# lighttransport/nanort

Measured on AMD Instinct MI355X. Metric: Mrays/s (primary + 1-bounce) at 1920x1080, 1M-tri mesh; BVH build ms, higher is better.
Workload: dtype f32; 1 GPU; C3: Plane(1000,500) = 1,000,000 triangles fp32; 1920x1080 objrender-camera primaries + 1 cosine bounce per hit (2073600 + 2055142 rays per GPU per step); parallelism=replicated BVH, interleaved image rows per GPU

## Files before the change

include/nanort_hip.h:

```cpp
#ifndef NANORT_HIP_H_
#define NANORT_HIP_H_

#include <stddef.h>
#include <stdint.h>

#ifdef __cplusplus
extern "C" {
#endif

#define NRT_API __attribute__((visibility("default")))

typedef int nrt_status;
enum {
  NRT_OK = 0,
  NRT_ERR_INVALID = 1,
  NRT_ERR_EMPTY = 2,
  NRT_ERR_DEVICE = 3,
  NRT_ERR_PRECISION = 4
};

typedef struct nrt_ctx nrt_ctx;


typedef struct {
// ... 92 lines not shown
#endif


NRT_API nrt_status nrtCreate(int device, nrt_ctx **out);
NRT_API void nrtDestroy(nrt_ctx *ctx);
NRT_API const char *nrtLastError(const nrt_ctx *ctx);
NRT_API const char *nrtVersion(void);

NRT_API nrt_status nrtHostAlloc(size_t bytes, void **out);
NRT_API void nrtHostFree(void *p);

NRT_API nrt_status nrtSetMesh_f32(nrt_ctx *ctx, const float *vertices, size_t vertex_stride_bytes,
                                  const uint32_t *faces, uint32_t num_faces);
NRT_API nrt_status nrtSetMesh_f64(nrt_ctx *ctx, const double *vertices, size_t vertex_stride_bytes,
                                  const uint32_t *faces, uint32_t num_faces);

NRT_API nrt_status nrtOccludedBatch_f32(nrt_ctx *ctx, const nrt_ray_f32 *rays, uint64_t num_rays,
                                        const nrt_trace_options *options, uint8_t *mask_out);
NRT_API nrt_status nrtOccludedBatch_f64(nrt_ctx *ctx, const nrt_ray_f64 *rays, uint64_t num_rays,
                                        const nrt_trace_options *options, uint8_t *mask_out);
NRT_API nrt_status nrtOccludedBatchDevice_f32(nrt_ctx *ctx, const nrt_ray_f32 *d_rays, uint64_t num_rays,
                                              const nrt_trace_options *options, uint8_t *d_mask_out, void *hip_stream);
NRT_API nrt_status nrtOccludedBatchDevice_f64(nrt_ctx *ctx, const nrt_ray_f64 *d_rays, uint64_t num_rays,
                                              const nrt_trace_options *options, uint8_t *d_mask_out, void *hip_stream);

#define NRT_MAX_MULTIHIT 64u
NRT_API nrt_status nrtMultiHitTraverseBatch_f32(nrt_ctx *ctx, const nrt_ray_f32 *rays, uint64_t num_rays, uint32_t max_hits,
                                                const nrt_trace_options *options, nrt_hit_f32 *hits_out, uint32_t *counts_out);
NRT_API nrt_status nrtMultiHitTraverseBatch_f64(nrt_ctx *ctx, const nrt_ray_f64 *rays, uint64_t num_rays, uint32_t max_hits,
                                                const nrt_trace_options *options, nrt_hit_f64 *hits_out, uint32_t *counts_out);
// ... 155 lines not shown
```

nanort_amd/accel.py:

```python
import ctypes

import numpy as np

from . import capi
from .wire import (
    BUILD_OPTIONS_F32,
    BUILD_OPTIONS_F64,
    BUILD_STATS,
    TRACE_OPTIONS,
    hit_dtype,
    node_dtype,
    ray_dtype,
    suffix,
)


def _p(a):
    return None if a is None else a.ctypes.data_as(ctypes.c_void_p)


class TriangleMesh:

    def __init__(self, vertices, faces, vertex_stride_bytes=None):
        self.vertices = np.ascontiguousarray(vertices)
# ... 79 lines not shown
        if isinstance(mesh, SphereGeometry):
            if self.real != np.float32:
                raise TypeError("sphere primitives are fp32 (as the reference example)")
            self._check(self._L.nrtSetSpheres_f32(self._h, _p(mesh.centers), _p(mesh.radii), mesh.num_spheres))
            self._mesh = mesh
            return
        if mesh.vertices.dtype != self.real:
            raise TypeError("mesh precision %s != accel precision %s" % (mesh.vertices.dtype, self.real))
        self._check(
            getattr(self._L, "nrtSetMesh_" + self._s)(
                self._h, _p(mesh.vertices), mesh.vertex_stride_bytes, _p(mesh.faces), mesh.num_faces
            )
        )
        self._mesh = mesh

    def Build(self, num_primitives, mesh, options=None):
        if num_primitives != mesh.num_faces:
            if isinstance(mesh, CylinderGeometry):
                mesh = CylinderGeometry(mesh.endpoints[:num_primitives], mesh.radii[:num_primitives], mesh.test_cap)
            elif isinstance(mesh, SphereGeometry):
                mesh = SphereGeometry(mesh.centers[:num_primitives], mesh.radii[:num_primitives])
            else:
                mesh = TriangleMesh(mesh.vertices, mesh.faces[:num_primitives], mesh.vertex_stride_bytes)
        self.SetMesh(mesh)
        if options is not None:
            want = BUILD_OPTIONS_F32 if self.real == np.float32 else BUILD_OPTIONS_F64
            options = np.asarray(options, dtype=want).reshape(1)
        nn = ctypes.c_uint64(0)
        st = getattr(self._L, "nrtBuild_" + self._s)(self._h, _p(options), _p(self._stats.reshape(1)), ctypes.byref(nn))
        if st == capi.NRT_ERR_EMPTY:
            return False
        self._check(st)
        return True

    def GetStatistics(self):
        return self._stats.copy()

    def LastBuildMs(self):
        return float(self._L.nrtLastBuildMs(self._h))
# ... 335 lines not shown
```

nanort_amd/capi.py:

```python
import ctypes
import os

_HERE = os.path.dirname(os.path.abspath(__file__))
LIB_PATH = os.path.join(_HERE, "lib", "libnanort_hip_prof.so" if os.environ.get("NRT_USE_PROF_LIB") == "1" else "libnanort_hip.so")

NRT_OK, NRT_ERR_INVALID, NRT_ERR_EMPTY, NRT_ERR_DEVICE, NRT_ERR_PRECISION = 0, 1, 2, 3, 4

SYMBOLS = [
    "nrtCreate", "nrtDestroy", "nrtLastError", "nrtVersion",
    "nrtSetMesh_f32", "nrtSetMesh_f64", "nrtSetSpheres_f32",
    "nrtSetCylinders_f32", "nrtTraverseBatchCylinders_f32", "nrtTraverseBatchCylindersDevice_f32",
    "nrtBuild_f32", "nrtBuild_f64",
    "nrtGetTree_f32", "nrtGetTree_f64", "nrtTreeSize", "nrtGetTreeBounds_f32", "nrtGetTreeBounds_f64",
    "nrtSetTree_f32", "nrtSetTree_f64",
    "nrtTraverseBatch_f32", "nrtTraverseBatch_f64",
    "nrtTraverseBatchDevice_f32", "nrtTraverseBatchDevice_f64", "nrtTraverseBatchesDevice_f32", "nrtTraverseBatchesDevice_f64", "nrtTraverseBatches_f32", "nrtTraverseBatches_f64",
    "nrtTraverseBatchMulti_f32", "nrtTraverseBatchMulti_f64", "nrtDeviceCount",
    "nrtTraverseCountDevice_f32", "nrtTraverseCountDevice_f64",
    "nrtOccludedBatch_f32", "nrtOccludedBatch_f64", "nrtOccludedBatchDevice_f32", "nrtOccludedBatchDevice_f64",
    "nrtMultiHitTraverseBatch_f32", "nrtMultiHitTraverseBatch_f64", "nrtMultiHitTraverseBatchDevice_f32", "nrtMultiHitTraverseBatchDevice_f64",
    "nrtRefit_f32", "nrtRefit_f64", "nrtRefitDevice_f32", "nrtRefitDevice_f64",
    "nrtLastTraverseMs", "nrtSetLaunchTiming", "nrtSetTunable", "nrtGetTunable", "nrtLastBuildMs", "nrtLastKernelName", "nrtHostAlloc", "nrtHostFree",
    "nrtGroupUniqueId", "nrtGroupCreate", "nrtGroupCreateRanked", "nrtGroupDestroy", "nrtGroupLastError", "nrtGroupSetTunable", "nrtGroupInfo",
    "nrtGroupTileRays", "nrtGroupTraverseGather_f32", "nrtGroupTraverseGather_f64", "nrtGroupTraverseGatherTiles_f32", "nrtGroupTraverseGatherTiles_f64", "nrtGroupSynchronize", "nrtGroupLastTraffic",
    "nrtSceneCreate", "nrtSceneDestroy", "nrtSceneLastError", "nrtSceneAddNode_f32", "nrtSceneCommit", "nrtSceneNodeState_f32",
# ... 35 lines not shown
    L = ctypes.CDLL(LIB_PATH, mode=ctypes.RTLD_GLOBAL)
    vp, u32, u64, sz, i32 = ctypes.c_void_p, ctypes.c_uint32, ctypes.c_uint64, ctypes.c_size_t, ctypes.c_int
    L.nrtCreate.argtypes = [i32, ctypes.POINTER(vp)]
    L.nrtCreate.restype = i32
    L.nrtDestroy.argtypes = [vp]
    L.nrtDestroy.restype = None
    L.nrtLastError.argtypes = [vp]
    L.nrtLastError.restype = ctypes.c_char_p
    L.nrtVersion.argtypes = []
    L.nrtVersion.restype = ctypes.c_char_p
    L.nrtTreeSize.argtypes = [vp, ctypes.POINTER(u64), ctypes.POINTER(u64)]
    L.nrtTreeSize.restype = i32
    for s in ("f32", "f64"):
        f = getattr(L, "nrtSetMesh_" + s)
        f.argtypes = [vp, vp, sz, vp, u32]
        f.restype = i32
        f = getattr(L, "nrtBuild_" + s)
        f.argtypes = [vp, vp, vp, ctypes.POINTER(u64)]
        f.restype = i32
        f = getattr(L, "nrtGetTree_" + s)
        f.argtypes = [vp, vp, vp]
        f.restype = i32
        f = getattr(L, "nrtSetTree_" + s)
        f.argtypes = [vp, vp, u64, vp, u64]
        f.restype = i32
        f = getattr(L, "nrtTraverseBatch_" + s)
        f.argtypes = [vp, vp, u64, vp, vp, vp]
        f.restype = i32
        f = getattr(L, "nrtTraverseBatchDevice_" + s)
        f.argtypes = [vp, vp, u64, vp, vp, vp, vp]
# ... 85 lines not shown
```

nanort_amd/csrc/api.hip:

```cpp
#include <hip/hip_runtime.h>
#include <stdarg.h>
#include <stdio.h>
#include <stdlib.h>
#include <string.h>
#include <ctype.h>
#include <math.h>
#include <cmath>

#include <algorithm>
#include <atomic>
#include <chrono>
#include <mutex>
#include <thread>
#include <string>
#include <vector>

#include "common.h"
#ifdef NRT_PROF
#include "../../include/nanort_hip_prof.h"
#endif

namespace nrt {
template <typename T>
hipError_t launch_traverse(const TraverseArgs<T> &, unsigned grid, bool count, int lds_stack, hipStream_t);
template <typename T>
int traverse_blocks_per_cu(int lds_stack);
// ... 29 lines not shown
size_t refit_plan_bytes(uint32_t tree_depth, uint64_t num_nodes);
template <typename T>
hipError_t launch_refit_plan(const typename Wire<T>::Node *nodes, uint64_t num_nodes, uint32_t num_branch_records, uint32_t tree_depth,
                             uint32_t root_is_branch, uint32_t *plan, hipStream_t s);
template <typename T>
hipError_t launch_refit(const void *src, size_t stride, bool aligned, uint32_t nv, T *verts, const uint32_t *faces, const uint32_t *indices,
                        typename Wire<T>::Node *nodes, uint64_t num_nodes, uint32_t num_branch_records, uint32_t tree_depth,
                        const uint32_t *plan, hipStream_t s);
hipError_t launch_cylinder_segments(const float *verts, const float *radii, const uint32_t *seg_off, uint32_t n, float *seg_verts,
                                    float *seg_radii, uint32_t *seg_prim, hipStream_t s);
}

using namespace nrt;

static thread_local std::string g_create_error;

struct nrt_ctx {
  int device = 0;
  hipStream_t stream = nullptr;
  std::string err;
  int prec = 0;
  int num_cus = 256;

  int prim_kind = kPrimTriangles;
  uint32_t cyl_test_cap = 1;
  DevBuf b_seg_verts, b_seg_radii, b_seg_prim, b_seg_off;
  uint32_t num_segs = 0;
  int cyl_split = 32;
  int cyl_seg_radii = 8;
  DevBuf b_verts, b_radii, b_faces;
// ... 62 lines not shown
  unsigned static_pct = 16;
  unsigned static_bands = 8;
  unsigned static_slice_groups = 2;
  unsigned max_blocks_per_cu = 0;
  int wide = 1, wide_stack = 10;
  int wide4 = 1;
  int wide4_big_ok = 1;
  int order4 = 0;
  int leaf_compact = 1;
  int dyn_head = 1;
  int wide_scramble = 0;
  unsigned wide4_blocks_per_cu = 0;
  unsigned wide_blocks_per_cu = 0, sphere_blocks_per_cu = 0;
  unsigned multihit_blocks_per_cu = 0;

  hipEvent_t ev_b0 = nullptr, ev_b1 = nullptr;
  hipEvent_t ev_build_state = nullptr;
  void *build_state = nullptr;
  int last_timed_slot = -1;
  int launch_timing = 0;
  bool have_build_time = false;
  float segment_ms = 0.f;
  const char *last_kernel = "";
};

static nrt_status fail(nrt_ctx *c, nrt_status st, const char *fmt, ...) {
  char buf[512];
  va_list ap;
  va_start(ap, fmt);
  vsnprintf(buf, sizeof(buf), fmt, ap);
// ... 75 lines not shown
    if (e != hipSuccess) return e;
  }
  return hipStreamSynchronize(c->stream);
}

static void free_tree(nrt_ctx *c) {
  c->generation++;
  c->d_wide = nullptr;
  c->d_wide4 = nullptr;
  c->d_nodes = nullptr;
  c->d_indices = nullptr;
  c->d_tris = nullptr;
  c->num_nodes = c->num_indices = 0;
  c->tree_depth = 0;
  c->refit_planned = false;
}

static void free_mesh(nrt_ctx *c) {
  c->d_verts = nullptr;
  c->d_faces = nullptr;
  c->d_radii = nullptr;
  c->num_faces = c->num_verts = 0;
  c->num_segs = 0;
}

struct TunableDesc {
  const char *name;
  long long lo, hi;
  long long (*get)(const nrt_ctx *);
  void (*set)(nrt_ctx *, long long);
};
#define NRT_TUNABLE(name_, lo_, hi_, field_, type_)                                                          \
  {name_, lo_, hi_, [](const nrt_ctx *c) -> long long { return (long long)c->field_; },                      \
   [](nrt_ctx *c, long long v) { c->field_ = (type_)v; }}
static const TunableDesc kTunables[] = {
    NRT_TUNABLE("refill_min", 1, 64, refill_min, unsigned),
    NRT_TUNABLE("trav_min", 1, 64, trav_min, unsigned),
    NRT_TUNABLE("trav_min4", 1, 64, trav_min4, unsigned),
    NRT_TUNABLE("f64_row_fetch", 0, 1, f64_row_fetch, int),
    NRT_TUNABLE("leaf_min", 1, 64, leaf_min, unsigned),
    NRT_TUNABLE("chunk_tail_pct", 0, 100, chunk_tail_pct, unsigned),
    NRT_TUNABLE("parts", 1, kMaxParts, num_parts, unsigned),
    NRT_TUNABLE("static_pct", 0, 100, static_pct, unsigned),
    NRT_TUNABLE("static_bands", 1, 64, static_bands, unsigned),
    NRT_TUNABLE("static_slice_groups", 1, 64, static_slice_groups, unsigned),
    NRT_TUNABLE("blocks_per_cu", 0, 8, max_blocks_per_cu, unsigned),
    NRT_TUNABLE("debug", 0, 0x7FFFFFFF, debug_flags, unsigned),
    NRT_TUNABLE("morton", 0, 1, morton, int),
    NRT_TUNABLE("cyl_split", 1, 64, cyl_split, int),
    NRT_TUNABLE("cyl_seg_radii", 1, 1024, cyl_seg_radii, int),
#ifdef NRT_PROF
    NRT_TUNABLE("subtree_rows", 0, 1, subtree_rows, int),
#endif
    NRT_TUNABLE("wide", 0, 1, wide, int),
    NRT_TUNABLE("wide4_big", 0, 2, wide4_big_ok, int),
    NRT_TUNABLE("wide4", 0, 1, wide4, int),
    NRT_TUNABLE("leaf_compact", 0, 1, leaf_compact, int),
    NRT_TUNABLE("dyn_head", 0, 1, dyn_head, int),
    NRT_TUNABLE("order4", 0, 1, order4, int),
    NRT_TUNABLE("launch_timing", 0, 1, launch_timing, int),
    NRT_TUNABLE("host_pipeline", 0, 1, host_pipeline, int),
    NRT_TUNABLE("wide_scramble", 0, 1, wide_scramble, int),
// ... 45 lines not shown
  int ndev = 0;
  hipError_t e = hipGetDeviceCount(&ndev);
  if (e != hipSuccess || ndev <= 0)
    return fail(nullptr, NRT_ERR_DEVICE, "nrtCreate: no HIP device visible (%s)",
                e == hipSuccess ? "count == 0" : hipGetErrorString(e));
  if (device < 0 || device >= ndev)
    return fail(nullptr, NRT_ERR_INVALID, "nrtCreate: device %d out of range [0,%d)", device, ndev);
  nrt_ctx *c = new nrt_ctx();
  c->device = device;
  if ((e = hipSetDevice(device)) != hipSuccess ||
      (e = hipStreamCreateWithFlags(&c->stream, hipStreamNonBlocking)) != hipSuccess ||
      (e = hipEventCreate(&c->ev_b0)) != hipSuccess || (e = hipEventCreate(&c->ev_b1)) != hipSuccess ||
      (e = hipEventCreateWithFlags(&c->ev_build_state, hipEventDisableTiming)) != hipSuccess ||
      (e = hipEventCreateWithFlags(&c->ev_refit, hipEventDisableTiming)) != hipSuccess ||
      (e = hipHostMalloc(&c->build_state, kBuildPinnedBytes, hipHostMallocDefault)) != hipSuccess ||
      (e = hipMalloc((void **)&c->d_counters, 16 * sizeof(unsigned long long))) != hipSuccess) {
    fail(nullptr, NRT_ERR_DEVICE, "nrtCreate: %s", hipGetErrorString(e));
    nrtDestroy(c);
    return NRT_ERR_DEVICE;
  }
  for (nrt_ctx::LaunchSlot &sl : c->slots) {
    if ((e = hipMalloc((void **)&sl.d_cursor, 2 * kCursorStrideWords * 4 * kMaxParts)) != hipSuccess ||
        (e = hipMemset(sl.d_cursor, 0, 2 * kCursorStrideWords * 4 * kMaxParts)) != hipSuccess ||
        (e = hipEventCreateWithFlags(&sl.done, hipEventDisableTiming)) != hipSuccess ||
        (e = hipEventCreate(&sl.t0)) != hipSuccess || (e = hipEventCreate(&sl.t1)) != hipSuccess ||
        (e = hipHostMalloc((void **)&sl.h_done, sizeof(DoneRec), hipHostMallocPortable | hipHostMallocMapped | hipHostMallocCoherent)) != hipSuccess ||
        (e = hipHostGetDevicePointer((void **)&sl.d_done, sl.h_done, 0)) != hipSuccess ||
        (e = hipMalloc((void **)&sl.d_count, sizeof(DoneCount))) != hipSuccess ||
        (e = hipMemset(sl.d_count, 0, sizeof(DoneCount))) != hipSuccess ||
        (e = hipMemset((char *)sl.d_count + offsetof(DoneCount, t_begin), 0xFF, sizeof(unsigned long long))) != hipSuccess) {
// ... 32 lines not shown
    if (sl.spill.p) (void)hipFree(sl.spill.p);
    if (sl.spill_tmin.p) (void)hipFree(sl.spill_tmin.p);
    if (sl.cyl_hits.p) (void)hipFree(sl.cyl_hits.p);
    if (sl.cyl_bits.p) (void)hipFree(sl.cyl_bits.p);
    if (sl.done) (void)hipEventDestroy(sl.done);
    if (sl.t0) (void)hipEventDestroy(sl.t0);
    if (sl.t1) (void)hipEventDestroy(sl.t1);
  }
  free_tree(c);
  free_mesh(c);
  DevBuf *bufs[] = {&c->b_verts, &c->b_radii, &c->b_faces, &c->st_rays, &c->st_hits, &c->st_mask, &c->b_nodes, &c->b_indices, &c->b_tris, &c->b_wide, &c->b_wide4, &c->b_wide_scratch, &c->b_build_ws, &c->b_wave_clock, &c->b_seg_verts, &c->b_seg_radii, &c->b_seg_prim, &c->b_seg_off, &c->b_refit_plan, &c->b_refit_stage};
  for (DevBuf *b : bufs)
    if (b->p) (void)hipFree(b->p);
  if (c->d_counters) (void)hipFree(c->d_counters);
  if (c->build_state) (void)hipHostFree(c->build_state);
  hipEvent_t evs[] = {c->ev_b0, c->ev_b1, c->ev_build_state, c->ev_refit};
  for (hipEvent_t ev : evs)
    if (ev) (void)hipEventDestroy(ev);
  for (int k = 0; k < 2; k++)
    for (hipEvent_t e : {c->ev_in[k], c->ev_tr[k], c->ev_out[k]})
      if (e) (void)hipEventDestroy(e);
  if (c->copy_in) (void)hipStreamDestroy(c->copy_in);
  if (c->copy_out) (void)hipStreamDestroy(c->copy_out);
  if (c->stream) (void)hipStreamDestroy(c->stream);
  delete c;
}

const char *nrtLastError(const nrt_ctx *c) { return c ? c->err.c_str() : g_create_error.c_str(); }

}

template <typename T>
static nrt_status set_mesh(nrt_ctx *c, const T *vertices, size_t stride, const uint32_t *faces,
                           uint32_t num_faces) {
  if (!c) return NRT_ERR_INVALID;
  if (c->prec != 0 && c->prec != (int)sizeof(T))
    return fail(c, NRT_ERR_PRECISION, "nrtSetMesh: context already holds a %s mesh",
                c->prec == 4 ? "f32" : "f64");
  if (num_faces && (!vertices || !faces)) return fail(c, NRT_ERR_INVALID, "nrtSetMesh: NULL mesh pointer");
  if (stride < 3 * sizeof(T) && num_faces)
    return fail(c, NRT_ERR_INVALID, "nrtSetMesh: vertex stride %zu < %zu", stride, 3 * sizeof(T));
  NRT_RANGE("nrtSetMesh (compaction + upload)");
  HIPCHK(c, hipSetDevice(c->device));
  HIPCHK(c, wait_for_launches(c));
  free_tree(c);
  free_mesh(c);
  c->prec = (int)sizeof(T);
  c->prim_kind = kPrimTriangles;
  c->num_faces = num_faces;
  if (num_faces == 0) return NRT_OK;
  uint32_t maxv = 0;
  const size_t ni = 3 * (size_t)num_faces;
  for (size_t i = 0; i < ni; i++) maxv = faces[i] > maxv ? faces[i] : maxv;
  const uint32_t nv = maxv + 1;
  c->num_verts = nv;
  const T *src = vertices;
  std::vector<T> tight;
  if (stride != 3 * sizeof(T)) {
    tight.resize(3 * (size_t)nv);
    const unsigned char *base = reinterpret_cast<const unsigned char *>(vertices);
    for (uint32_t v = 0; v < nv; v++) {
      const T *p = reinterpret_cast<const T *>(base + (size_t)v * stride);
      tight[3 * (size_t)v + 0] = p[0];
      tight[3 * (size_t)v + 1] = p[1];
      tight[3 * (size_t)v + 2] = p[2];
    }
    src = tight.data();
  }
  nrt_status st;
  if ((st = ensure(c, c->b_verts, 3 * (size_t)nv * sizeof(T))) || (st = ensure(c, c->b_faces, ni * sizeof(uint32_t)))) return st;
  c->d_verts = c->b_verts.p;
  c->d_faces = (uint32_t *)c->b_faces.p;
  HIPCHK(c, hipMemcpy(c->d_verts, src, 3 * (size_t)nv * sizeof(T), hipMemcpyHostToDevice));
  HIPCHK(c, hipMemcpy(c->d_faces, faces, ni * sizeof(uint32_t), hipMemcpyHostToDevice));
  return NRT_OK;
}

template <typename T>
static nrt_status set_spheres(nrt_ctx *c, const T *centers, const T *radii, uint32_t n) {
  if (!c) return NRT_ERR_INVALID;
  if (c->prec != 0 && c->prec != (int)sizeof(T))
    return fail(c, NRT_ERR_PRECISION, "nrtSetSpheres: context already holds %s primitives", c->prec == 4 ? "f32" : "f64");
  if (n && (!centers || !radii)) return fail(c, NRT_ERR_INVALID, "nrtSetSpheres: NULL pointer");
  HIPCHK(c, hipSetDevice(c->device));
  HIPCHK(c, wait_for_launches(c));
  free_tree(c);
  free_mesh(c);
  c->prec = (int)sizeof(T);
  c->prim_kind = kPrimSpheres;
  c->num_faces = n;
// ... 173 lines not shown
  c->min_leaf_count = min_leaf;
  c->root_is_branch = nodes[0].flag == 0 ? 1u : 0u;
  c->tree_nested = nested;
  c->num_branch_records = 0;
  for (uint64_t i = 0; i < num_nodes; i++)
    if (nodes[i].flag == 0) c->num_branch_records++;
  nrt_status st;
  if ((st = ensure(c, c->b_nodes, num_nodes * sizeof(typename Wire<T>::Node)))) return st;
  if ((st = ensure(c, c->b_indices, std::max<uint64_t>(1, num_indices) * sizeof(uint32_t)))) return st;
  c->d_nodes = c->b_nodes.p;
  c->d_indices = (uint32_t *)c->b_indices.p;
  HIPCHK(c, hipMemcpy(c->d_nodes, nodes, num_nodes * sizeof(typename Wire<T>::Node), hipMemcpyHostToDevice));
  HIPCHK(c, hipMemcpy(c->d_indices, indices, num_indices * sizeof(uint32_t), hipMemcpyHostToDevice));
  if ((st = finish_tree<T>(c, c->stream))) return st;
  HIPCHK(c, hipStreamSynchronize(c->stream));
  return NRT_OK;
}

template <typename T>
static nrt_status get_tree(nrt_ctx *c, typename Wire<T>::Node *nodes_out, uint32_t *indices_out) {
  if (!c) return NRT_ERR_INVALID;
  if (c->prec != (int)sizeof(T)) return fail(c, NRT_ERR_PRECISION, "nrtGetTree: precision mismatch");
  if (!c->d_nodes) return fail(c, NRT_ERR_INVALID, "nrtGetTree: no tree");
  NRT_RANGE("nrtGetTree (read-back)");
  HIPCHK(c, hipSetDevice(c->device));
  HIPCHK(c, refit_host_wait(c));
  HIPCHK(c, hipStreamSynchronize(c->stream));
  if (nodes_out)
    HIPCHK(c, hipMemcpy(nodes_out, c->d_nodes, c->num_nodes * sizeof(typename Wire<T>::Node), hipMemcpyDeviceToHost));
  if (indices_out)
    HIPCHK(c, hipMemcpy(indices_out, c->d_indices, c->num_indices * sizeof(uint32_t), hipMemcpyDeviceToHost));
  return NRT_OK;
}

template <typename T>
static nrt_status get_tree_bounds(nrt_ctx *c, T *bmin, T *bmax) {
  if (!c || !bmin || !bmax) return NRT_ERR_INVALID;
  if (c->prec != (int)sizeof(T)) return fail(c, NRT_ERR_PRECISION, "nrtGetTreeBounds: precision mismatch");
  if (!c->d_nodes) return fail(c, NRT_ERR_INVALID, "nrtGetTreeBounds: no tree");
  HIPCHK(c, hipSetDevice(c->device));
  HIPCHK(c, refit_host_wait(c));
  HIPCHK(c, hipStreamSynchronize(c->stream));
  T box[6];
  HIPCHK(c, hipMemcpy(box, c->d_nodes, sizeof(box), hipMemcpyDeviceToHost));
  for (int k = 0; k < 3; k++) {
    bmin[k] = box[k];
    bmax[k] = box[3 + k];
  }
  return NRT_OK;
}

template <typename T>
static nrt_status build(nrt_ctx *c, const typename Wire<T>::BuildOptions *opt, nrt_build_stats *stats_out,
                        uint64_t *num_nodes_out) {
// ... 36 lines not shown
  }
  c->num_nodes = res.num_nodes;
  c->tree_depth = res.max_depth;
  c->max_leaf_count = res.max_leaf_count;
  c->num_branch_records = res.num_branches;
  c->root_is_branch = res.num_nodes > 1 ? 1u : 0u;
  c->min_leaf_count = 1;
  c->tree_nested = 1;
  NRT_RANGE_PUSH("build: WideNode / Wide4Node records");
  fst = finish_wide<T>(c, c->stream);
  NRT_RANGE_POP();
  if (fst) {
    free_tree(c);
    return fst;
  }
  HIPCHK(c, hipEventRecord(c->ev_b1, c->stream));
  HIPCHK(c, hipEventSynchronize(c->ev_b1));
  c->have_build_time = true;
  float ms = 0.f;
  HIPCHK(c, hipEventElapsedTime(&ms, c->ev_b0, c->ev_b1));
  c->stats.max_tree_depth = res.max_depth;
  c->stats.num_leaf_nodes = res.num_leaves;
  c->stats.num_branch_nodes = res.num_branches;
  c->stats.build_secs = (ms + (segs ? c->segment_ms : 0.f)) * 1e-3f;
  if (stats_out) *stats_out = c->stats;
  if (num_nodes_out) *num_nodes_out = c->num_nodes;
  return NRT_OK;
}

template <typename T>
static nrt_status refit(nrt_ctx *c, const T *vertices, size_t stride, bool device, hipStream_t s) {
  const char *fn = device ? "nrtRefitDevice" : "nrtRefit";
// ... 18 lines not shown
  if (!device && nv) {
    if ((st = ensure(c, c->b_refit_stage, block))) return st;
    HIPCHK(c, hipMemcpyAsync(c->b_refit_stage.p, vertices, block, hipMemcpyHostToDevice, s));
    src = c->b_refit_stage.p;
  }
  if (!c->refit_planned) {
    if ((st = ensure(c, c->b_refit_plan, refit_plan_bytes(c->tree_depth, c->num_nodes)))) return st;
    HIPCHK(c, launch_refit_plan<T>((const typename Wire<T>::Node *)c->d_nodes, c->num_nodes, c->num_branch_records, c->tree_depth,
                                   c->root_is_branch, (uint32_t *)c->b_refit_plan.p, s));
    c->refit_planned = true;
  }
  hipError_t e = launch_refit<T>(src, stride, stride % sizeof(T) == 0, nv, (T *)c->d_verts, c->d_faces, c->d_indices,
                                 (typename Wire<T>::Node *)c->d_nodes, c->num_nodes, c->num_branch_records, c->tree_depth,
                                 (const uint32_t *)c->b_refit_plan.p, s);
  c->tree_nested = 1;
  if (e == hipSuccess && (st = finish_tree<T>(c, s))) e = hipErrorUnknown;
  if (e == hipSuccess && !device) e = hipStreamSynchronize(s);
  if (e == hipSuccess && device) {
    std::lock_guard<std::mutex> lock(c->launch_mutex);
    if ((e = hipEventRecord(c->ev_refit, s)) == hipSuccess) c->refit_pending = true;
  }
  if (e != hipSuccess) {
    const std::string why = st ? c->err : std::string(hipGetErrorString(e));
    (void)hipStreamSynchronize(s);
    free_tree(c);
    free_mesh(c);
    return fail(c, NRT_ERR_DEVICE, "%s: %s (the context's tree and primitives were dropped: set the mesh again)", fn, why.c_str());
  }
  c->generation++;
  return NRT_OK;
// ... 636 lines not shown
  return multihit_device<double>(c, r, n, k, o, h, cnt, (hipStream_t)s);
}

nrt_status nrtRefit_f32(nrt_ctx *c, const float *v, size_t stride) { return refit<float>(c, v, stride, false, nullptr); }
nrt_status nrtRefit_f64(nrt_ctx *c, const double *v, size_t stride) { return refit<double>(c, v, stride, false, nullptr); }
nrt_status nrtRefitDevice_f32(nrt_ctx *c, const float *v, size_t stride, void *s) { return refit<float>(c, v, stride, true, (hipStream_t)s); }
nrt_status nrtRefitDevice_f64(nrt_ctx *c, const double *v, size_t stride, void *s) { return refit<double>(c, v, stride, true, (hipStream_t)s); }

nrt_status nrtSetMesh_f32(nrt_ctx *c, const float *v, size_t stride, const uint32_t *f, uint32_t nf) {
  return set_mesh<float>(c, v, stride, f, nf);
}
nrt_status nrtSetMesh_f64(nrt_ctx *c, const double *v, size_t stride, const uint32_t *f, uint32_t nf) {
  return set_mesh<double>(c, v, stride, f, nf);
}

nrt_status nrtSetCylinders_f32(nrt_ctx *c, const float *endpoints, const float *radii, uint32_t n, int test_cap) {
  return set_cylinders(c, endpoints, radii, n, test_cap);
}

nrt_status nrtTraverseBatchCylindersDevice_f32(nrt_ctx *c, const nrt_ray_f32 *r, uint64_t n, const nrt_trace_options *o,
                                               nrt_cyl_hit_f32 *h, uint8_t *m, void *s) {
  if (!c) return NRT_ERR_INVALID;
  if (n && !h) return fail(c, NRT_ERR_INVALID, "nrtTraverseBatchCylindersDevice: NULL hits");
  return traverse_device<float>(c, r, n, o, nullptr, m, (hipStream_t)s, false, true, h);
}

nrt_status nrtTraverseBatchCylinders_f32(nrt_ctx *c, const nrt_ray_f32 *rays, uint64_t n, const nrt_trace_options *opt,
                                         nrt_cyl_hit_f32 *hits, uint8_t *mask) {
  if (!c) return NRT_ERR_INVALID;
  if (n == 0) return NRT_OK;
// ... 206 lines not shown
```

Baseline: 6804 Mrays/s.

## Pipeline mesh upload through pinned staging ring and add device-side mesh input

Replaces the synchronous pageable hipMemcpy mesh upload with a chunked, multi-threaded pinned staging ring that overlaps host copying and max-index scanning with async H2D transfers. Adds nrtSetMeshDevice entry points that compact vertices and validate faces on the GPU, deferring the bounds check until the build publishes it through mapped host memory. Also caches the root box so GetTreeBounds skips a device sync. This targets BVH build and upload time, not traversal throughput, at the cost of a thread pool, busy-wait spinning and more complex error paths.

```diff
diff --git a/include/nanort_hip.h b/include/nanort_hip.h
--- a/include/nanort_hip.h
+++ b/include/nanort_hip.h
@@ -130,6 +130,10 @@
                                   const uint32_t *faces, uint32_t num_faces);
 NRT_API nrt_status nrtSetMesh_f64(nrt_ctx *ctx, const double *vertices, size_t vertex_stride_bytes,
                                   const uint32_t *faces, uint32_t num_faces);
+NRT_API nrt_status nrtSetMeshDevice_f32(nrt_ctx *ctx, const float *d_vertices, size_t vertex_stride_bytes, uint32_t num_vertices,
+                                        const uint32_t *d_faces, uint32_t num_faces, void *hip_stream);
+NRT_API nrt_status nrtSetMeshDevice_f64(nrt_ctx *ctx, const double *d_vertices, size_t vertex_stride_bytes, uint32_t num_vertices,
+                                        const uint32_t *d_faces, uint32_t num_faces, void *hip_stream);
 
 NRT_API nrt_status nrtOccludedBatch_f32(nrt_ctx *ctx, const nrt_ray_f32 *rays, uint64_t num_rays,
                                         const nrt_trace_options *options, uint8_t *mask_out);
diff --git a/nanort_amd/accel.py b/nanort_amd/accel.py
--- a/nanort_amd/accel.py
+++ b/nanort_amd/accel.py
@@ -117,6 +117,32 @@
         )
         self._mesh = mesh
 
+    def SetMeshDevice(self, d_vertices, d_faces, stream=None):
+        import torch
+
+        want = torch.float32 if self.real == np.float32 else torch.float64
+        if d_vertices.dtype != want:
+            raise TypeError("vertex dtype %s != accel precision %s" % (d_vertices.dtype, self.real))
+        if d_vertices.dim() != 2 or d_vertices.shape[1] < 3 or d_vertices.stride(1) != 1:
+            raise ValueError("vertices must be [nv, k >= 3] with stride(1) == 1")
+        if d_faces.dtype not in (torch.int32, getattr(torch, "uint32", torch.int32)) or not d_faces.is_contiguous() or d_faces.numel() % 3:
+            raise ValueError("faces must be a contiguous 32-bit integer tensor of 3 indices per face")
+        for t in (d_vertices, d_faces):
+            if t.device.type != "cuda" or t.device.index != self.device:
+                raise ValueError("the mesh must live on cuda:%d" % self.device)
+        if stream is None:
+            stream = torch.cuda.current_stream(self.device).cuda_stream
+        elif hasattr(stream, "cuda_stream"):
+            stream = stream.cuda_stream
+        stride = d_vertices.stride(0) * d_vertices.element_size()
+        self._check(getattr(self._L, "nrtSetMeshDevice_" + self._s)(
+            self._h, d_vertices.data_ptr(), stride, d_vertices.shape[0], d_faces.data_ptr(), d_faces.numel() // 3, stream))
+        self._mesh = None
+
+    def BuildDevice(self, d_vertices, d_faces, options=None, stream=None):
+        self.SetMeshDevice(d_vertices, d_faces, stream)
+        return self._build(options)
+
     def Build(self, num_primitives, mesh, options=None):
         if num_primitives != mesh.num_faces:
             if isinstance(mesh, CylinderGeometry):
@@ -126,6 +152,9 @@
             else:
                 mesh = TriangleMesh(mesh.vertices, mesh.faces[:num_primitives], mesh.vertex_stride_bytes)
         self.SetMesh(mesh)
+        return self._build(options)
+
+    def _build(self, options):
         if options is not None:
             want = BUILD_OPTIONS_F32 if self.real == np.float32 else BUILD_OPTIONS_F64
             options = np.asarray(options, dtype=want).reshape(1)
diff --git a/nanort_amd/capi.py b/nanort_amd/capi.py
--- a/nanort_amd/capi.py
+++ b/nanort_amd/capi.py
@@ -8,7 +8,7 @@
 
 SYMBOLS = [
     "nrtCreate", "nrtDestroy", "nrtLastError", "nrtVersion",
-    "nrtSetMesh_f32", "nrtSetMesh_f64", "nrtSetSpheres_f32",
+    "nrtSetMesh_f32", "nrtSetMesh_f64", "nrtSetMeshDevice_f32", "nrtSetMeshDevice_f64", "nrtSetSpheres_f32",
     "nrtSetCylinders_f32", "nrtTraverseBatchCylinders_f32", "nrtTraverseBatchCylindersDevice_f32",
     "nrtBuild_f32", "nrtBuild_f64",
     "nrtGetTree_f32", "nrtGetTree_f64", "nrtTreeSize", "nrtGetTreeBounds_f32", "nrtGetTreeBounds_f64",
@@ -74,6 +74,9 @@
     for s in ("f32", "f64"):
         f = getattr(L, "nrtSetMesh_" + s)
         f.argtypes = [vp, vp, sz, vp, u32]
+        f.restype = i32
+        f = getattr(L, "nrtSetMeshDevice_" + s)
+        f.argtypes = [vp, vp, sz, u32, vp, u32, vp]
         f.restype = i32
         f = getattr(L, "nrtBuild_" + s)
         f.argtypes = [vp, vp, vp, ctypes.POINTER(u64)]
diff --git a/nanort_amd/csrc/api.hip b/nanort_amd/csrc/api.hip
--- a/nanort_amd/csrc/api.hip
+++ b/nanort_amd/csrc/api.hip
@@ -10,6 +10,8 @@
 #include <algorithm>
 #include <atomic>
 #include <chrono>
+#include <condition_variable>
+#include <functional>
 #include <mutex>
 #include <thread>
 #include <string>
@@ -69,6 +71,68 @@
 using namespace nrt;
 
 static thread_local std::string g_create_error;
+
+struct StagePool {
+  static constexpr int kSlots = 8;
+  std::vector<std::thread> threads;
+  std::mutex m;
+  std::condition_variable cv;
+  bool quit = false;
+  std::atomic<uint64_t> job_seq{0};
+  std::function<uint32_t(size_t, void *)> fill;
+  size_t nchunks = 0;
+  void **ring = nullptr;
+  std::atomic<long long> ready_for[kSlots], filled[kSlots];
+  std::atomic<uint32_t> maxv{0};
+  std::atomic<int> left{0};
+  std::atomic<bool> abort{false};
+
+  void work(unsigned w, unsigned W) {
+    uint64_t seen = 0;
+    for (;;) {
+      for (int spin = 0; spin < 20000 && job_seq.load(std::memory_order_acquire) == seen; spin++) {
+      }
+      {
+        std::unique_lock<std::mutex> lock(m);
+        cv.wait(lock, [&] { return quit || job_seq.load(std::memory_order_acquire) != seen; });
+        if (quit) return;
+        seen = job_seq.load(std::memory_order_acquire);
+      }
+      uint32_t mine = 0;
+      for (size_t k = w; k < nchunks && !abort.load(std::memory_order_relaxed); k += W) {
+        const int slot = (int)(k % kSlots);
+        while (ready_for[slot].load(std::memory_order_acquire) != (long long)k)
+          if (abort.load(std::memory_order_relaxed)) break;
+        if (abort.load(std::memory_order_relaxed)) break;
+        const uint32_t got = fill(k, ring[slot]);
+        mine = got > mine ? got : mine;
+        filled[slot].store((long long)k + 1, std::memory_order_release);
+      }
+      uint32_t cur = maxv.load(std::memory_order_relaxed);
+      while (mine > cur && !maxv.compare_exchange_weak(cur, mine, std::memory_order_relaxed)) {
+      }
+      left.fetch_sub(1, std::memory_order_release);
+    }
+  }
+  void start(unsigned W) {
+    for (unsigned w = 0; w < W; w++) threads.emplace_back([this, w, W] { work(w, W); });
+  }
+  void stop() {
+    {
+      std::lock_guard<std::mutex> lock(m);
+      quit = true;
+    }
+    cv.notify_all();
+    for (std::thread &t : threads) t.join();
+    threads.clear();
+  }
+};
+
+struct HostNote {
+  uint32_t max_index;
+  uint32_t pad;
+  unsigned char root_box[6 * sizeof(double)];
+};
 
 struct nrt_ctx {
   int device = 0;
@@ -161,6 +225,21 @@
   unsigned wide_blocks_per_cu = 0, sphere_blocks_per_cu = 0;
   unsigned multihit_blocks_per_cu = 0;
 
+  static constexpr int kRing = 8;
+  void *ring[kRing] = {};
+  size_t ring_bytes = 0;
+  hipEvent_t ring_ev[kRing] = {};
+  bool ring_busy[kRing] = {};
+  unsigned upload_chunk_kib = 2048;
+  unsigned upload_threads = 3;
+  StagePool *pool = nullptr;
+  HostNote *h_note = nullptr, *d_note = nullptr;
+  uint32_t *d_mesh_max = nullptr;
+  hipEvent_t ev_mesh = nullptr;
+  bool mesh_check_pending = false;
+  bool root_box_valid = false;
+  unsigned char root_box[6 * sizeof(double)];
+
   hipEvent_t ev_b0 = nullptr, ev_b1 = nullptr;
   hipEvent_t ev_build_state = nullptr;
   void *build_state = nullptr;
@@ -266,6 +345,7 @@
   c->num_nodes = c->num_indices = 0;
   c->tree_depth = 0;
   c->refit_planned = false;
+  c->root_box_valid = false;
 }
 
 static void free_mesh(nrt_ctx *c) {
@@ -274,6 +354,7 @@
   c->d_radii = nullptr;
   c->num_faces = c->num_verts = 0;
   c->num_segs = 0;
+  c->mesh_check_pending = false;
 }
 
 struct TunableDesc {
@@ -298,6 +379,8 @@
     NRT_TUNABLE("static_slice_groups", 1, 64, static_slice_groups, unsigned),
     NRT_TUNABLE("blocks_per_cu", 0, 8, max_blocks_per_cu, unsigned),
     NRT_TUNABLE("debug", 0, 0x7FFFFFFF, debug_flags, unsigned),
+    NRT_TUNABLE("upload_chunk", 4, 1 << 20, upload_chunk_kib, unsigned),
+    NRT_TUNABLE("upload_threads", 0, 8, upload_threads, unsigned),
     NRT_TUNABLE("morton", 0, 1, morton, int),
     NRT_TUNABLE("cyl_split", 1, 64, cyl_split, int),
     NRT_TUNABLE("cyl_seg_radii", 1, 1024, cyl_seg_radii, int),
@@ -373,6 +456,11 @@
       (e = hipEventCreateWithFlags(&c->ev_build_state, hipEventDisableTiming)) != hipSuccess ||
       (e = hipEventCreateWithFlags(&c->ev_refit, hipEventDisableTiming)) != hipSuccess ||
       (e = hipHostMalloc(&c->build_state, kBuildPinnedBytes, hipHostMallocDefault)) != hipSuccess ||
+      (e = hipHostMalloc((void **)&c->h_note, sizeof(HostNote), hipHostMallocPortable | hipHostMallocMapped | hipHostMallocCoherent)) != hipSuccess ||
+      (e = hipHostGetDevicePointer((void **)&c->d_note, c->h_note, 0)) != hipSuccess ||
+      (e = hipMalloc((void **)&c->d_mesh_max, sizeof(uint32_t))) != hipSuccess ||
+      (e = hipMemset(c->d_mesh_max, 0, sizeof(uint32_t))) != hipSuccess ||
+      (e = hipEventCreateWithFlags(&c->ev_mesh, hipEventDisableTiming)) != hipSuccess ||
       (e = hipMalloc((void **)&c->d_counters, 16 * sizeof(unsigned long long))) != hipSuccess) {
     fail(nullptr, NRT_ERR_DEVICE, "nrtCreate: %s", hipGetErrorString(e));
     nrtDestroy(c);
@@ -435,7 +523,17 @@
     if (b->p) (void)hipFree(b->p);
   if (c->d_counters) (void)hipFree(c->d_counters);
   if (c->build_state) (void)hipHostFree(c->build_state);
-  hipEvent_t evs[] = {c->ev_b0, c->ev_b1, c->ev_build_state, c->ev_refit};
+  if (c->pool) {
+    c->pool->stop();
+    delete c->pool;
+  }
+  if (c->h_note) (void)hipHostFree(c->h_note);
+  if (c->d_mesh_max) (void)hipFree(c->d_mesh_max);
+  for (int k = 0; k < nrt_ctx::kRing; k++) {
+    if (c->ring[k]) (void)hipHostFree(c->ring[k]);
+    if (c->ring_ev[k]) (void)hipEventDestroy(c->ring_ev[k]);
+  }
+  hipEvent_t evs[] = {c->ev_b0, c->ev_b1, c->ev_build_state, c->ev_refit, c->ev_mesh};
   for (hipEvent_t ev : evs)
     if (ev) (void)hipEventDestroy(ev);
   for (int k = 0; k < 2; k++)
@@ -451,6 +549,136 @@
 
 }
 
+static nrt_status ring_take(nrt_ctx *c, int slot, void **out) {
+  if (c->ring_busy[slot]) {
+    hipError_t q;
+    while ((q = hipEventQuery(c->ring_ev[slot])) == hipErrorNotReady) {
+    }
+    if (q != hipSuccess) return fail(c, NRT_ERR_DEVICE, "nrtSetMesh: staging copy failed: %s", hipGetErrorString(q));
+    c->ring_busy[slot] = false;
+  }
+  *out = c->ring[slot];
+  return NRT_OK;
+}
+static nrt_status ring_ensure(nrt_ctx *c, size_t bytes) {
+  if (bytes <= c->ring_bytes && c->ring[0]) return NRT_OK;
+  for (int k = 0; k < nrt_ctx::kRing; k++) {
+    void *dummy;
+    nrt_status st = ring_take(c, k, &dummy);
+    if (st) return st;
+    if (c->ring[k]) (void)hipHostFree(c->ring[k]);
+    c->ring[k] = nullptr;
+  }
+  c->ring_bytes = 0;
+  for (int k = 0; k < nrt_ctx::kRing; k++) {
+    HIPCHK(c, hipHostMalloc(&c->ring[k], bytes, hipHostMallocDefault));
+    if (!c->ring_ev[k]) HIPCHK(c, hipEventCreateWithFlags(&c->ring_ev[k], hipEventDisableTiming));
+  }
+  c->ring_bytes = bytes;
+  return NRT_OK;
+}
+static nrt_status ring_send(nrt_ctx *c, int slot, void *dst, size_t bytes) {
+  HIPCHK(c, hipMemcpyAsync(dst, c->ring[slot], bytes, hipMemcpyHostToDevice, c->stream));
+  HIPCHK(c, hipEventRecord(c->ring_ev[slot], c->stream));
+  c->ring_busy[slot] = true;
+  return NRT_OK;
+}
+
+static std::vector<size_t> chunk_cuts(size_t n, size_t most) {
+  std::vector<size_t> cut(1, 0);
+  most = std::max<size_t>(most, 1);
+  for (size_t size = std::max<size_t>(most / 8, std::min<size_t>(most, 8192)); cut.back() < n; size = std::min(most, 2 * size))
+    cut.push_back(std::min(n, cut.back() + size));
+  return cut;
+}
+
+static nrt_status upload_chunks(nrt_ctx *c, size_t nchunks, size_t slot_bytes, const std::function<uint32_t(size_t, void *)> &fill,
+                                const std::function<void *(size_t)> &dst_of, const std::function<size_t(size_t)> &bytes_of, uint32_t *max_out) {
+  static_assert(StagePool::kSlots == nrt_ctx::kRing, "one state word per ring slot");
+  *max_out = 0;
+  if (nchunks == 0) return NRT_OK;
+  size_t largest = 0;
+  for (size_t k = 0; k < nchunks; k++) largest = std::max(largest, bytes_of(k));
+  nrt_status st = ring_ensure(c, (std::min(slot_bytes, largest) + 0xFFFF) & ~(size_t)0xFFFF);
+  if (st) return st;
+  uint32_t maxv = 0;
+  const unsigned W = (unsigned)std::min<size_t>(c->upload_threads, nchunks);
+  if (W < 2) {
+    for (size_t k = 0; k < nchunks && !st; k++) {
+      const int slot = (int)(k % nrt_ctx::kRing);
+      void *stage;
+      if ((st = ring_take(c, slot, &stage))) break;
+      const uint32_t m = fill(k, stage);
+      maxv = m > maxv ? m : maxv;
+      st = ring_send(c, slot, dst_of(k), bytes_of(k));
+    }
+    *max_out = maxv;
+    return st;
+  }
+  if (c->pool && c->pool->threads.size() != c->upload_threads) {
+    c->pool->stop();
+    delete c->pool;
+    c->pool = nullptr;
+  }
+  if (!c->pool) {
+    c->pool = new StagePool();
+    c->pool->start(c->upload_threads);
+  }
+  StagePool &p = *c->pool;
+  long long inflight[nrt_ctx::kRing];
+  for (int s = 0; s < nrt_ctx::kRing; s++) {
+    inflight[s] = (long long)s - nrt_ctx::kRing;
+    p.ready_for[s].store(c->ring_busy[s] ? -1 : (long long)s, std::memory_order_relaxed);
+    p.filled[s].store(0, std::memory_order_relaxed);
+  }
+  p.fill = fill;
+  p.nchunks = nchunks;
+  p.ring = c->ring;
+  p.maxv.store(0, std::memory_order_relaxed);
+  p.abort.store(false, std::memory_order_relaxed);
+  p.left.store((int)p.threads.size(), std::memory_order_relaxed);
+  {
+    std::lock_guard<std::mutex> lock(p.m);
+    p.job_seq.fetch_add(1, std::memory_order_release);
+  }
+  p.cv.notify_all();
+  for (size_t next = 0; next < nchunks && !st;) {
+    const int slot = (int)(next % nrt_ctx::kRing);
+    if (p.filled[slot].load(std::memory_order_acquire) == (long long)next + 1) {
+      st = ring_send(c, slot, dst_of(next), bytes_of(next));
+      inflight[slot] = (long long)next;
+      next++;
+      continue;
+    }
+    for (int s = 0; s < nrt_ctx::kRing && !st; s++) {
+      if (!c->ring_busy[s]) continue;
+      const hipError_t q = hipEventQuery(c->ring_ev[s]);
+      if (q == hipErrorNotReady) continue;
+      if (q != hipSuccess) {
+        st = fail(c, NRT_ERR_DEVICE, "nrtSetMesh: staging copy failed: %s", hipGetErrorString(q));
+        break;
+      }
+      c->ring_busy[s] = false;
+      p.ready_for[s].store(inflight[s] + nrt_ctx::kRing, std::memory_order_release);
+    }
+  }
+  if (st) p.abort.store(true, std::memory_order_relaxed);
+  while (p.left.load(std::memory_order_acquire) != 0) {
+  }
+  *max_out = p.maxv.load(std::memory_order_relaxed);
+  return st;
+}
+
+static inline uint32_t copy_max_u32(uint32_t *__restrict__ dst, const uint32_t *__restrict__ src, size_t n) {
+  uint32_t m = 0;
+  for (size_t i = 0; i < n; i++) {
+    const uint32_t v = src[i];
+    dst[i] = v;
+    m = v > m ? v : m;
+  }
+  return m;
+}
+
 template <typename T>
 static nrt_status set_mesh(nrt_ctx *c, const T *vertices, size_t stride, const uint32_t *faces,
                            uint32_t num_faces) {
@@ -461,7 +689,7 @@
   if (num_faces && (!vertices || !faces)) return fail(c, NRT_ERR_INVALID, "nrtSetMesh: NULL mesh pointer");
   if (stride < 3 * sizeof(T) && num_faces)
     return fail(c, NRT_ERR_INVALID, "nrtSetMesh: vertex stride %zu < %zu", stride, 3 * sizeof(T));
-  NRT_RANGE("nrtSetMesh (compaction + upload)");
+  NRT_RANGE("nrtSetMesh (staging + upload)");
   HIPCHK(c, hipSetDevice(c->device));
   HIPCHK(c, wait_for_launches(c));
   free_tree(c);
@@ -470,31 +698,142 @@
   c->prim_kind = kPrimTriangles;
   c->num_faces = num_faces;
   if (num_faces == 0) return NRT_OK;
-  uint32_t maxv = 0;
   const size_t ni = 3 * (size_t)num_faces;
-  for (size_t i = 0; i < ni; i++) maxv = faces[i] > maxv ? faces[i] : maxv;
+  const size_t chunk_bytes = std::max<size_t>((size_t)c->upload_chunk_kib << 10, 3 * sizeof(T));
+  nrt_status st;
+  if ((st = ensure(c, c->b_faces, ni * sizeof(uint32_t)))) return st;
+  c->d_faces = (uint32_t *)c->b_faces.p;
+  uint32_t maxv = 0, unused = 0;
+  uint32_t *d_faces = c->d_faces;
+  const std::vector<size_t> fcut = chunk_cuts(ni, chunk_bytes / sizeof(uint32_t));
+  const size_t *fc = fcut.data();
+  st = upload_chunks(
+      c, fcut.size() - 1, chunk_bytes, [=](size_t k, void *stage) { return copy_max_u32((uint32_t *)stage, faces + fc[k], fc[k + 1] - fc[k]); },
+      [=](size_t k) { return (void *)(d_faces + fc[k]); }, [=](size_t k) { return (fc[k + 1] - fc[k]) * sizeof(uint32_t); }, &maxv);
+  if (!st && maxv == 0xFFFFFFFFu) st = fail(c, NRT_ERR_INVALID, "nrtSetMesh: vertex index 0xFFFFFFFF");
   const uint32_t nv = maxv + 1;
+  if (!st) st = ensure(c, c->b_verts, 3 * (size_t)nv * sizeof(T));
+  if (!st) {
+    T *d_verts = (T *)c->b_verts.p;
+    const std::vector<size_t> vcut = chunk_cuts(nv, chunk_bytes / (3 * sizeof(T)));
+    const size_t *vc = vcut.data();
+    const unsigned char *base = reinterpret_cast<const unsigned char *>(vertices);
+    st = upload_chunks(
+        c, vcut.size() - 1, chunk_bytes,
+        [=](size_t k, void *stage) {
+          const size_t at = vc[k], n = vc[k + 1] - at;
+          if (stride == 3 * sizeof(T)) {
+            memcpy(stage, base + at * stride, n * 3 * sizeof(T));
+          } else {
+            T *out = (T *)stage;
+            for (size_t v = 0; v < n; v++) {
+              T p[3];
+              memcpy(p, base + (at + v) * stride, sizeof(p));
+              out[3 * v + 0] = p[0];
+              out[3 * v + 1] = p[1];
+              out[3 * v + 2] = p[2];
+            }
+          }
+          return 0u;
+        },
+        [=](size_t k) { return (void *)(d_verts + 3 * vc[k]); }, [=](size_t k) { return (vc[k + 1] - vc[k]) * 3 * sizeof(T); }, &unused);
+  }
+  if (st) {
+    c->d_faces = nullptr;
+    c->num_faces = 0;
+    return st;
+  }
+  c->d_verts = c->b_verts.p;
   c->num_verts = nv;
-  const T *src = vertices;
-  std::vector<T> tight;
-  if (stride != 3 * sizeof(T)) {
-    tight.resize(3 * (size_t)nv);
-    const unsigned char *base = reinterpret_cast<const unsigned char *>(vertices);
-    for (uint32_t v = 0; v < nv; v++) {
-      const T *p = reinterpret_cast<const T *>(base + (size_t)v * stride);
-      tight[3 * (size_t)v + 0] = p[0];
-      tight[3 * (size_t)v + 1] = p[1];
-      tight[3 * (size_t)v + 2] = p[2];
-    }
-    src = tight.data();
-  }
+  return NRT_OK;
+}
+
+__global__ void k_publish_note(const uint32_t *__restrict__ root, uint32_t box_words, const uint32_t *__restrict__ mesh_max, HostNote *note) {
+  uint32_t *box = reinterpret_cast<uint32_t *>(note->root_box);
+  if (threadIdx.x < box_words) __hip_atomic_store(&box[threadIdx.x], root[threadIdx.x], __ATOMIC_RELAXED, __HIP_MEMORY_SCOPE_SYSTEM);
+  if (threadIdx.x == 63u) __hip_atomic_store(&note->max_index, *mesh_max, __ATOMIC_RELAXED, __HIP_MEMORY_SCOPE_SYSTEM);
+}
+
+__global__ __launch_bounds__(256) void k_copy_faces_max(const uint32_t *__restrict__ src, uint32_t *__restrict__ dst, size_t n, uint32_t nv,
+                                                        uint32_t *max_out) {
+  uint32_t m = 0;
+  for (size_t i = (size_t)blockIdx.x * 256u + threadIdx.x; i < n; i += (size_t)gridDim.x * 256u) {
+    const uint32_t v = src[i];
+    m = v > m ? v : m;
+    dst[i] = v < nv ? v : 0u;
+  }
+  for (int off = 32; off > 0; off >>= 1) {
+    const uint32_t o = (uint32_t)__shfl_xor((int)m, off, 64);
+    m = o > m ? o : m;
+  }
+  if ((threadIdx.x & 63u) == 0u && m != 0u) atomicMax(max_out, m);
+}
+template <typename T>
+__global__ __launch_bounds__(256) void k_compact_verts(const T *__restrict__ src, size_t stride_elems, uint32_t nv, T *__restrict__ dst) {
+  const size_t i = (size_t)blockIdx.x * 256u + threadIdx.x;
+  if (i >= 3 * (size_t)nv) return;
+  dst[i] = src[(i / 3) * stride_elems + i % 3];
+}
+
+template <typename T>
+static nrt_status set_mesh_device(nrt_ctx *c, const T *d_vertices, size_t stride, uint32_t num_vertices, const uint32_t *d_faces,
+                                  uint32_t num_faces, hipStream_t s) {
+  if (!c) return NRT_ERR_INVALID;
+  if (c->prec != 0 && c->prec != (int)sizeof(T))
+    return fail(c, NRT_ERR_PRECISION, "nrtSetMeshDevice: context already holds a %s mesh", c->prec == 4 ? "f32" : "f64");
+  if (num_faces && (!d_vertices || !d_faces)) return fail(c, NRT_ERR_INVALID, "nrtSetMeshDevice: NULL mesh pointer");
+  if (stride < 3 * sizeof(T) && num_faces)
+    return fail(c, NRT_ERR_INVALID, "nrtSetMeshDevice: vertex stride %zu < %zu", stride, 3 * sizeof(T));
+  if (num_faces && (stride % sizeof(T) != 0 || (uintptr_t)d_vertices % sizeof(T) != 0 || (uintptr_t)d_faces % sizeof(uint32_t) != 0))
+    return fail(c, NRT_ERR_INVALID, "nrtSetMeshDevice: vertex stride %zu or a pointer not aligned to its element size", stride);
+  if (num_faces && num_vertices == 0) return fail(c, NRT_ERR_INVALID, "nrtSetMeshDevice: %u faces over 0 vertices", num_faces);
+  NRT_RANGE("nrtSetMeshDevice");
+  HIPCHK(c, hipSetDevice(c->device));
+  HIPCHK(c, wait_for_launches(c));
+  free_tree(c);
+  free_mesh(c);
+  c->prec = (int)sizeof(T);
+  c->prim_kind = kPrimTriangles;
+  c->num_faces = num_faces;
+  if (num_faces == 0) return NRT_OK;
+  const size_t ni = 3 * (size_t)num_faces;
   nrt_status st;
-  if ((st = ensure(c, c->b_verts, 3 * (size_t)nv * sizeof(T))) || (st = ensure(c, c->b_faces, ni * sizeof(uint32_t)))) return st;
+  if ((st = ensure(c, c->b_verts, 3 * (size_t)num_vertices * sizeof(T))) || (st = ensure(c, c->b_faces, ni * sizeof(uint32_t)))) {
+    c->num_faces = 0;
+    return st;
+  }
+  hipError_t e = hipMemsetAsync(c->d_mesh_max, 0, sizeof(uint32_t), s);
+  if (e == hipSuccess) {
+    hipLaunchKernelGGL(k_copy_faces_max, dim3((unsigned)std::min<size_t>((ni + 255) / 256, 4096)), dim3(256), 0, s, d_faces,
+                       (uint32_t *)c->b_faces.p, ni, num_vertices, c->d_mesh_max);
+    hipLaunchKernelGGL((k_compact_verts<T>), dim3((unsigned)((3 * (size_t)num_vertices + 255) / 256)), dim3(256), 0, s, d_vertices,
+                       stride / sizeof(T), num_vertices, (T *)c->b_verts.p);
+    e = hipGetLastError();
+  }
+  if (e == hipSuccess) e = hipEventRecord(c->ev_mesh, s);
+  if (e == hipSuccess) e = hipStreamWaitEvent(c->stream, c->ev_mesh, 0);
+  if (e != hipSuccess) {
+    (void)hipStreamSynchronize(s);
+    c->num_faces = 0;
+    return fail(c, NRT_ERR_DEVICE, "nrtSetMeshDevice: %s", hipGetErrorString(e));
+  }
   c->d_verts = c->b_verts.p;
   c->d_faces = (uint32_t *)c->b_faces.p;
-  HIPCHK(c, hipMemcpy(c->d_verts, src, 3 * (size_t)nv * sizeof(T), hipMemcpyHostToDevice));
-  HIPCHK(c, hipMemcpy(c->d_faces, faces, ni * sizeof(uint32_t), hipMemcpyHostToDevice));
-  return NRT_OK;
+  c->num_verts = num_vertices;
+  c->mesh_check_pending = true;
+  return NRT_OK;
+}
+
+static nrt_status mesh_check(nrt_ctx *c, const char *fn, bool in_note) {
+  if (!c->mesh_check_pending) return NRT_OK;
+  c->mesh_check_pending = false;
+  uint32_t maxv = *(volatile const uint32_t *)&c->h_note->max_index;
+  const uint32_t nv = c->num_verts;
+  if (!in_note) HIPCHK(c, hipMemcpy(&maxv, c->d_mesh_max, sizeof(maxv), hipMemcpyDeviceToHost));
+  if (maxv < nv) return NRT_OK;
+  free_tree(c);
+  free_mesh(c);
+  return fail(c, NRT_ERR_INVALID, "%s: the device mesh's faces name vertex %u, the vertex count given was %u (the mesh was dropped)", fn, maxv, nv);
 }
 
 template <typename T>
@@ -698,7 +1037,7 @@
   HIPCHK(c, hipMemcpy(c->d_indices, indices, num_indices * sizeof(uint32_t), hipMemcpyHostToDevice));
   if ((st = finish_tree<T>(c, c->stream))) return st;
   HIPCHK(c, hipStreamSynchronize(c->stream));
-  return NRT_OK;
+  return mesh_check(c, "nrtSetTree", false);
 }
 
 template <typename T>
@@ -722,6 +1061,15 @@
   if (!c || !bmin || !bmax) return NRT_ERR_INVALID;
   if (c->prec != (int)sizeof(T)) return fail(c, NRT_ERR_PRECISION, "nrtGetTreeBounds: precision mismatch");
   if (!c->d_nodes) return fail(c, NRT_ERR_INVALID, "nrtGetTreeBounds: no tree");
+  if (c->root_box_valid) {
+    T box[6];
+    memcpy(box, c->root_box, sizeof(box));
+    for (int k = 0; k < 3; k++) {
+      bmin[k] = box[k];
+      bmax[k] = box[3 + k];
+    }
+    return NRT_OK;
+  }
   HIPCHK(c, hipSetDevice(c->device));
   HIPCHK(c, refit_host_wait(c));
   HIPCHK(c, hipStreamSynchronize(c->stream));
@@ -788,8 +1136,15 @@
     free_tree(c);
     return fst;
   }
+  static_assert(sizeof(c->h_note->root_box) >= 6 * sizeof(T) && sizeof(c->root_box) == sizeof(c->h_note->root_box), "root box");
+  hipLaunchKernelGGL(k_publish_note, dim3(1), dim3(64), 0, c->stream, (const uint32_t *)c->d_nodes, (uint32_t)(6 * sizeof(T) / sizeof(uint32_t)),
+                     (const uint32_t *)c->d_mesh_max, c->d_note);
+  HIPCHK(c, hipGetLastError());
   HIPCHK(c, hipEventRecord(c->ev_b1, c->stream));
   HIPCHK(c, hipEventSynchronize(c->ev_b1));
+  if ((fst = mesh_check(c, "nrtBuild", true))) return fst;
+  memcpy(c->root_box, c->h_note->root_box, 6 * sizeof(T));
+  c->root_box_valid = true;
   c->have_build_time = true;
   float ms = 0.f;
   HIPCHK(c, hipEventElapsedTime(&ms, c->ev_b0, c->ev_b1));
@@ -838,6 +1193,7 @@
                                  (typename Wire<T>::Node *)c->d_nodes, c->num_nodes, c->num_branch_records, c->tree_depth,
                                  (const uint32_t *)c->b_refit_plan.p, s);
   c->tree_nested = 1;
+  c->root_box_valid = false;
   if (e == hipSuccess && (st = finish_tree<T>(c, s))) e = hipErrorUnknown;
   if (e == hipSuccess && !device) e = hipStreamSynchronize(s);
   if (e == hipSuccess && device) {
@@ -1504,6 +1860,13 @@
   return set_mesh<double>(c, v, stride, f, nf);
 }
 
+nrt_status nrtSetMeshDevice_f32(nrt_ctx *c, const float *v, size_t stride, uint32_t nv, const uint32_t *f, uint32_t nf, void *s) {
+  return set_mesh_device<float>(c, v, stride, nv, f, nf, (hipStream_t)s);
+}
+nrt_status nrtSetMeshDevice_f64(nrt_ctx *c, const double *v, size_t stride, uint32_t nv, const uint32_t *f, uint32_t nf, void *s) {
+  return set_mesh_device<double>(c, v, stride, nv, f, nf, (hipStream_t)s);
+}
+
 nrt_status nrtSetCylinders_f32(nrt_ctx *c, const float *endpoints, const float *radii, uint32_t n, int test_cap) {
   return set_cylinders(c, endpoints, radii, n, test_cap);
 }
```

Measured after the change: 6815 Mrays/s (median of 6 runs). Within noise of the previous version (+0.2%).
